# isl-org/lang-seg

Hardware: AMD Instinct MI355X
Metric: images/sec at 480x480, ViT-L/16 + 150 ADE20K labels (higher is better)
Workload: dtype fp16; 1 GPU; BASELINE configs[1]: clip_vitl16_384 LSegNet.forward, 480x480, K=150 ADE20K labels, text tower recomputed every call; per_gpu_batch=36, global_batch=36, labels=150, parallelism=dp1 (batch sharded, no collectives)

## Files before the change

lang-seg_amd/csrc/attention.hip:

```cpp
#include <cstdlib>
#include <type_traits>

#include "ops.h"
#include "../../include/lseg_hip.h"

namespace lseg {

struct AttnArgs {
    const uint16_t* q; const uint16_t* k; const uint16_t* vt;
    uint16_t* out;
    float* lse2;
    int B, H, ntok, npad, causal;
    float scale_log2e;
    int prescaled;
};

namespace {

#ifndef ATTN_PROBE
#define ATTN_PROBE(i)
#define ATTN_PROBE_DECL
#define ATTN_PROBE_DUMP
#endif

template <typename T, int NW, int NS, bool PRE>
__global__ __launch_bounds__(64 * NW, NW == 8 ? 2 : 3) void lseg_attention_kernel(const AttnArgs a) {
    extern __shared__ __attribute__((aligned(16))) char smem[];
    constexpr int TILE = 8192, STAGE = 2 * TILE;
    const int tid = threadIdx.x, lane = tid & 63;
    const int w = __builtin_amdgcn_readfirstlane(tid >> 6);
    const int hi = lane >> 5, ql = lane & 31;
    const int nqb = (a.ntok + 32 * NW - 1) / (32 * NW), BH = a.B * a.H;
    const int L = blockIdx.x;
    int qb = L % nqb, bh = L / nqb;
    if ((BH & 7) == 0) {
        const int xcd = L & 7, idx = L >> 3;
        qb = idx % nqb;
        bh = (idx / nqb) * 8 + xcd;
    }
    const int q0 = (qb * NW + w) * 32;
    const uint16_t* Q = a.q + (size_t)bh * a.npad * 64;
    const uint16_t* K = a.k + (size_t)bh * a.npad * 64;
    const uint16_t* Vt = a.vt + (size_t)bh * 64 * a.npad;

    i32x4_t qf[4];
    {
        int qr = q0 + ql;
        if (qr > a.npad - 1) qr = a.npad - 1;
#pragma unroll
        for (int ks = 0; ks < 4; ++ks)
            qf[ks] = *reinterpret_cast<const i32x4_t*>(Q + (size_t)qr * 64 + ks * 16 + hi * 8);
    }

    int kv_end = a.ntok;
    if (a.causal) {
        const int qend = (qb + 1) * 32 * NW;
        kv_end = qend < a.ntok ? qend : a.ntok;
    }
    const int n_tiles = (kv_end + 63) >> 6;

    constexpr int SPW = 8 / NW;
    uint32_t k_off[SPW], v_off[SPW];
#pragma unroll
    for (int s = 0; s < SPW; ++s) {
        const int r = (s * NW + w) * 8 + (lane >> 3);
        const int ch = ((lane & 7) ^ swz(r)) << 3;
        k_off[s] = (uint32_t)(r * 64 + ch) * 2u;
        v_off[s] = (uint32_t)(r * a.npad + ch) * 2u;
    }
    auto issue = [&](int t, int stage) {
        char* sk = smem + stage * STAGE;
        char* sv = sk + TILE;
        const char* kb = uniform_ptr(reinterpret_cast<const char*>(K + (size_t)t * 64 * 64));
        const char* vb = uniform_ptr(reinterpret_cast<const char*>(Vt + (size_t)t * 64));
#pragma unroll
        for (int s = 0; s < SPW; ++s) {
            uint32_t ko = k_off[s], vo = v_off[s];
            asm volatile("" : "+v"(ko), "+v"(vo));
            glds_slab_off(kb, ko, sk + (s * NW + w) * 1024);
            glds_slab_off(vb, vo, sv + (s * NW + w) * 1024);
        }
    };

    f32x16_t o[2];
#pragma unroll
    for (int d = 0; d < 2; ++d)
#pragma unroll
        for (int r = 0; r < 16; ++r) o[d][r] = 0.f;
    float m_run = PRE ? 0.f : -1e30f, l_run = 0.f;
    f32x16_t lacc;
#pragma unroll
    for (int r = 0; r < 16; ++r) lacc[r] = 0.f;
    const int one2 = std::is_same<T, F16>::value ? 0x3C003C00 : 0x3F803F80;
    const i32x4_t ones = {one2, one2, one2, one2};
    const int qrow = q0 + ql;
    const bool live = q0 < a.ntok;

    issue(0, 0);
    if (NS == 3 && n_tiles > 1) issue(1, 1);
    ATTN_PROBE_DECL
    int st_cur = 0, st_nxt = NS - 1;
    for (int t = 0; t < n_tiles; ++t) {
        if (NS == 3 && t + 1 < n_tiles) __builtin_amdgcn_s_waitcnt((2 * SPW) | (7 << 4));
        else __builtin_amdgcn_s_waitcnt(0);
        __syncthreads();
        ATTN_PROBE(0)
        if (t + NS - 1 < n_tiles) issue(t + NS - 1, st_nxt);
        const int st_use = st_cur;
        st_nxt = st_cur;
        st_cur = st_cur + 1 == NS ? 0 : st_cur + 1;
        if (!live) continue;
        ATTN_PROBE(1)
        const char* sk = smem + st_use * STAGE;
        const char* sv = sk + TILE;

        {
            i32x4_t kf[8];
#pragma unroll
            for (int ks = 0; ks < 4; ++ks)
#pragma unroll
                for (int sub = 0; sub < 2; ++sub)
                    kf[ks * 2 + sub] = *reinterpret_cast<const i32x4_t*>(sk + tile_off(sub * 32 + ql, ks * 2 + hi));
            __builtin_amdgcn_sched_barrier(0);
            f32x16_t s[2];
            const float s_init = PRE ? -m_run : 0.f;
#pragma unroll
            for (int sub = 0; sub < 2; ++sub)
#pragma unroll
                for (int r = 0; r < 16; ++r) s[sub][r] = s_init;
#pragma unroll
            for (int ks = 0; ks < 4; ++ks)
#pragma unroll
                for (int sub = 0; sub < 2; ++sub) s[sub] = mfma32<T>(kf[ks * 2 + sub], qf[ks], s[sub]);
            i32x4_t vf[8];
#pragma unroll
            for (int sub = 0; sub < 2; ++sub)
#pragma unroll
                for (int s2 = 0; s2 < 2; ++s2)
#pragma unroll
                    for (int d = 0; d < 2; ++d)
                        vf[(sub * 2 + s2) * 2 + d] = *reinterpret_cast<const i32x4_t*>(sv + tile_off(d * 32 + ql, sub * 4 + s2 * 2 + hi));
            __builtin_amdgcn_sched_barrier(0);
            ATTN_PROBE(2)
            const bool need_mask = a.causal || (t * 64 + 64 > a.ntok);
            if (need_mask) {
#pragma unroll
                for (int sub = 0; sub < 2; ++sub)
#pragma unroll
                    for (int r = 0; r < 16; ++r) {
                        const int key = t * 64 + sub * 32 + (r & 3) + 8 * (r >> 2) + 4 * hi;
                        const bool ok = key < a.ntok && (!a.causal || key <= qrow);
                        s[sub][r] = ok ? s[sub][r] : -INFINITY;
                    }
            }
            float mx = -INFINITY;
#pragma unroll
            for (int sub = 0; sub < 2; ++sub)
#pragma unroll
                for (int r = 0; r < 16; ++r) mx = fmaxf(mx, s[sub][r]);
            {
                const auto sw = __builtin_amdgcn_permlane32_swap(__float_as_uint(mx), __float_as_uint(mx), false, false);
                mx = fmaxf(__uint_as_float(sw[0]), __uint_as_float(sw[1]));
            }
            ATTN_PROBE(3)
            float lsum = 0.f;
            if constexpr (!PRE) {
                mx *= a.scale_log2e;
                const float m_new = fmaxf(m_run, mx);
                const bool grew = !__all(m_new == m_run);
                float alpha = 1.0f;
                if (grew) alpha = __builtin_amdgcn_exp2f(m_run - m_new);
                m_run = m_new;
#pragma unroll
                for (int sub = 0; sub < 2; ++sub)
#pragma unroll
                    for (int r = 0; r < 16; ++r) {
                        const float p = __builtin_amdgcn_exp2f(fmaf(s[sub][r], a.scale_log2e, -m_new));
                        s[sub][r] = p;
                        lsum += p;
                    }
                l_run = l_run * alpha + lsum;
                if (grew) {
#pragma unroll
                    for (int d = 0; d < 2; ++d)
#pragma unroll
                        for (int r = 0; r < 16; ++r) o[d][r] *= alpha;
                }
            } else {
                constexpr float THR = 8.0f;
                if (t == 0 || __any(mx > THR)) {
                    const float delta = t == 0 ? mx : fmaxf(mx, 0.f);
                    const float alpha = __builtin_amdgcn_exp2f(-delta);
                    m_run += delta;
#pragma unroll
                    for (int sub = 0; sub < 2; ++sub)
#pragma unroll
                        for (int r = 0; r < 16; ++r) s[sub][r] -= delta;
                    if (t > 0) {
#pragma unroll
                        for (int d = 0; d < 2; ++d)
#pragma unroll
                            for (int r = 0; r < 16; ++r) o[d][r] *= alpha;
#pragma unroll
                        for (int r = 0; r < 16; ++r) lacc[r] *= alpha;
                    }
                }
#pragma unroll
                for (int sub = 0; sub < 2; ++sub)
#pragma unroll
                    for (int r = 0; r < 16; ++r) {
                        s[sub][r] = __builtin_amdgcn_exp2f(s[sub][r]);
                    }
            }
            i32x4_t pf[2][2];
#pragma unroll
            for (int sub = 0; sub < 2; ++sub)
#pragma unroll
                for (int s2 = 0; s2 < 2; ++s2) {
                    const uint32_t a0 = pack2<T>(s[sub][8 * s2 + 0], s[sub][8 * s2 + 1]);
                    const uint32_t a1 = pack2<T>(s[sub][8 * s2 + 2], s[sub][8 * s2 + 3]);
                    const uint32_t b0 = pack2<T>(s[sub][8 * s2 + 4], s[sub][8 * s2 + 5]);
                    const uint32_t b1 = pack2<T>(s[sub][8 * s2 + 6], s[sub][8 * s2 + 7]);
                    const auto w0 = __builtin_amdgcn_permlane32_swap(a0, b0, false, false);
                    const auto w1 = __builtin_amdgcn_permlane32_swap(a1, b1, false, false);
                    pf[sub][s2][0] = (int)w0[0]; pf[sub][s2][1] = (int)w1[0];
                    pf[sub][s2][2] = (int)w0[1]; pf[sub][s2][3] = (int)w1[1];
                }
            ATTN_PROBE(4)
#pragma unroll
            for (int sub = 0; sub < 2; ++sub)
#pragma unroll
                for (int s2 = 0; s2 < 2; ++s2) {
#pragma unroll
                    for (int d = 0; d < 2; ++d) o[d] = mfma32<T>(vf[(sub * 2 + s2) * 2 + d], pf[sub][s2], o[d]);
                    if constexpr (PRE) lacc = mfma32<T>(ones, pf[sub][s2], lacc);
                }
        }
        ATTN_PROBE(5)
    }
    ATTN_PROBE_DUMP

    const float l_tot = PRE ? lacc[0] : l_run + __shfl_xor(l_run, 32);
    const float inv = 1.0f / l_tot;
    if (a.lse2 && hi == 0 && qrow < a.ntok) a.lse2[(size_t)bh * a.npad + qrow] = m_run + __builtin_amdgcn_logf(l_tot);
    if (qrow < a.ntok) {
        const int b = bh / a.H, h = bh - b * a.H;
        uint16_t* orow = a.out + ((size_t)b * a.ntok + qrow) * (a.H * 64) + h * 64;
#pragma unroll
        for (int d = 0; d < 2; ++d)
#pragma unroll
            for (int g = 0; g < 4; g += 2) {
                const uint32_t ax = pack2<T>(o[d][g * 4 + 0] * inv, o[d][g * 4 + 1] * inv), ay = pack2<T>(o[d][g * 4 + 2] * inv, o[d][g * 4 + 3] * inv);
                const uint32_t bx = pack2<T>(o[d][g * 4 + 4] * inv, o[d][g * 4 + 5] * inv), by = pack2<T>(o[d][g * 4 + 6] * inv, o[d][g * 4 + 7] * inv);
                const auto sx = __builtin_amdgcn_permlane32_swap(ax, bx, false, false);
                const auto sy = __builtin_amdgcn_permlane32_swap(ay, by, false, false);
                *reinterpret_cast<uint4*>(orow + d * 32 + (g + hi) * 8) = make_uint4(sx[0], sy[0], sx[1], sy[1]);
            }
    }
}

}

int launch_attention(const void* q, const void* k, const void* vt, void* out, int B, int H, int ntok,
                     int npad, int dtype, int causal, float scale, hipStream_t stream) {
    return launch_attention_lse(q, k, vt, out, nullptr, B, H, ntok, npad, dtype, causal, scale, stream);
}

int launch_attention_lse(const void* q, const void* k, const void* vt, void* out, float* lse2, int B, int H, int ntok,
                         int npad, int dtype, int causal, float scale, hipStream_t stream) {
    return launch_attention_ex(q, k, vt, out, lse2, B, H, ntok, npad, dtype, causal, scale, 0, stream);
}

int launch_attention_ex(const void* q, const void* k, const void* vt, void* out, float* lse2, int B, int H, int ntok,
                        int npad, int dtype, int causal, float scale, int prescaled, hipStream_t stream) {
    if (npad % 128 != 0 || npad < ntok) return set_error(LSEG_ERR_INVALID, "attention: npad=%d must be a multiple of 128 and >= ntok=%d", npad, ntok);
    if (prescaled && causal) return set_error(LSEG_ERR_UNSUPPORTED, "attention: the pre-scaled form has no causal variant");
    AttnArgs a;
    a.q = (const uint16_t*)q; a.k = (const uint16_t*)k; a.vt = (const uint16_t*)vt; a.out = (uint16_t*)out;
    a.lse2 = lse2;
    a.B = B; a.H = H; a.ntok = ntok; a.npad = npad; a.causal = causal;
    a.scale_log2e = scale * 1.4426950408889634f;
    a.prescaled = prescaled;
    if (dtype != DT_BF16 && dtype != DT_F16) return set_error(LSEG_ERR_INVALID, "attention: dtype %d", dtype);
    int dev = 0;
    LSEG_HIP_TRY(hipGetDevice(&dev));
    const bool narrow = (long)((ntok + 127) / 128) * B * H < 2L * device_cu_count(dev) && !causal;
    const int nw = narrow ? 2 : 4;
    const size_t lds = (size_t)2 * 2 * 8192;
    dim3 grid(((ntok + 32 * nw - 1) / (32 * nw)) * B * H);
#define ATT(TT, NWV, PV) hipLaunchKernelGGL((lseg_attention_kernel<TT, NWV, 2, PV>), grid, dim3(64 * NWV), lds, stream, a)
#define ATT_T(NWV, PV) do { if (dtype == DT_BF16) ATT(BF16, NWV, PV); else ATT(F16, NWV, PV); } while (0)
    if (nw == 2) { if (prescaled) ATT_T(2, true); else ATT_T(2, false); }
    else { if (prescaled) ATT_T(4, true); else ATT_T(4, false); }
#undef ATT_T
#undef ATT
    LSEG_HIP_TRY(hipGetLastError());
    return 0;
}

}
```

Baseline: 1085 images/sec.

## Add persistent 64-row-per-wave pre-scaled attention kernel with ping-pong softmax overlap

Adds a persistent attention kernel for the pre-scaled, non-causal path. Each wave owns 64 query rows as two 32-row halves, and the schedule interleaves one half's softmax/exp work with the other half's QK and PV MFMAs. K/V tiles are shared through a 3-stage LDS pipeline, and the running-max rescale is skipped unless the new max exceeds a threshold. It is selected when there are enough work items per CU, with an env override; the intent is to hide VALU softmax latency behind matrix work and halve K/V LDS reads per query row. In exchange it adds register pressure (launch bound of 1 block per CU), a larger LDS footprint and lazy-rescale numerics, and leaves compile-time ablation macros in the old kernel that are off by default.

```diff
diff --git a/lang-seg_amd/csrc/attention.hip b/lang-seg_amd/csrc/attention.hip
--- a/lang-seg_amd/csrc/attention.hip
+++ b/lang-seg_amd/csrc/attention.hip
@@ -16,6 +16,10 @@
 };
 
 namespace {
+
+#ifndef ATTN_ABL
+#define ATTN_ABL 0
+#endif
 
 #ifndef ATTN_PROBE
 #define ATTN_PROBE(i)
@@ -100,6 +104,9 @@
     if (NS == 3 && n_tiles > 1) issue(1, 1);
     ATTN_PROBE_DECL
     int st_cur = 0, st_nxt = NS - 1;
+#if ATTN_ABL == 3
+    i32x4_t kf_keep[8], vf_keep[8];
+#endif
     for (int t = 0; t < n_tiles; ++t) {
         if (NS == 3 && t + 1 < n_tiles) __builtin_amdgcn_s_waitcnt((2 * SPW) | (7 << 4));
         else __builtin_amdgcn_s_waitcnt(0);
@@ -116,11 +123,24 @@
 
         {
             i32x4_t kf[8];
+#if ATTN_ABL == 3
+            if (!PRE || t == 0)
+#endif
 #pragma unroll
             for (int ks = 0; ks < 4; ++ks)
 #pragma unroll
                 for (int sub = 0; sub < 2; ++sub)
                     kf[ks * 2 + sub] = *reinterpret_cast<const i32x4_t*>(sk + tile_off(sub * 32 + ql, ks * 2 + hi));
+#if ATTN_ABL == 3
+            if (PRE) {
+                if (t == 0) {
+#pragma unroll
+                    for (int i = 0; i < 8; ++i) kf_keep[i] = kf[i];
+                }
+#pragma unroll
+                for (int i = 0; i < 8; ++i) kf[i] = kf_keep[i];
+            }
+#endif
             __builtin_amdgcn_sched_barrier(0);
             f32x16_t s[2];
             const float s_init = PRE ? -m_run : 0.f;
@@ -133,6 +153,9 @@
 #pragma unroll
                 for (int sub = 0; sub < 2; ++sub) s[sub] = mfma32<T>(kf[ks * 2 + sub], qf[ks], s[sub]);
             i32x4_t vf[8];
+#if ATTN_ABL == 3
+            if (!PRE || t == 0)
+#endif
 #pragma unroll
             for (int sub = 0; sub < 2; ++sub)
 #pragma unroll
@@ -140,8 +163,22 @@
 #pragma unroll
                     for (int d = 0; d < 2; ++d)
                         vf[(sub * 2 + s2) * 2 + d] = *reinterpret_cast<const i32x4_t*>(sv + tile_off(d * 32 + ql, sub * 4 + s2 * 2 + hi));
+#if ATTN_ABL == 3
+            if (PRE) {
+                if (t == 0) {
+#pragma unroll
+                    for (int i = 0; i < 8; ++i) vf_keep[i] = vf[i];
+                }
+#pragma unroll
+                for (int i = 0; i < 8; ++i) vf[i] = vf_keep[i];
+            }
+#endif
             __builtin_amdgcn_sched_barrier(0);
             ATTN_PROBE(2)
+#if ATTN_ABL == 2 || ATTN_ABL == 3
+            if (PRE) asm volatile("" : "+v"(s[0]), "+v"(s[1]));
+            if (!PRE) {
+#endif
             const bool need_mask = a.causal || (t * 64 + 64 > a.ntok);
             if (need_mask) {
 #pragma unroll
@@ -209,10 +246,29 @@
                 for (int sub = 0; sub < 2; ++sub)
 #pragma unroll
                     for (int r = 0; r < 16; ++r) {
+#if ATTN_ABL == 1
+                        float e;
+                        asm("v_mov_b32 %0, %1" : "=v"(e) : "v"(s[sub][r]));
+                        s[sub][r] = e;
+#else
                         s[sub][r] = __builtin_amdgcn_exp2f(s[sub][r]);
+#endif
                     }
             }
+#if ATTN_ABL == 2 || ATTN_ABL == 3
+            }
+#endif
             i32x4_t pf[2][2];
+#if ATTN_ABL == 3
+            if (PRE) {
+#pragma unroll
+                for (int sub = 0; sub < 2; ++sub)
+#pragma unroll
+                    for (int s2 = 0; s2 < 2; ++s2)
+#pragma unroll
+                        for (int i = 0; i < 4; ++i) pf[sub][s2][i] = (int)__float_as_uint(s[sub][8 * s2 + i]);
+            } else
+#endif
 #pragma unroll
             for (int sub = 0; sub < 2; ++sub)
 #pragma unroll
@@ -233,7 +289,7 @@
                 for (int s2 = 0; s2 < 2; ++s2) {
 #pragma unroll
                     for (int d = 0; d < 2; ++d) o[d] = mfma32<T>(vf[(sub * 2 + s2) * 2 + d], pf[sub][s2], o[d]);
-                    if constexpr (PRE) lacc = mfma32<T>(ones, pf[sub][s2], lacc);
+                    if constexpr (PRE && ATTN_ABL != 4) lacc = mfma32<T>(ones, pf[sub][s2], lacc);
                 }
         }
         ATTN_PROBE(5)
@@ -259,7 +315,252 @@
     }
 }
 
-}
+__device__ __forceinline__ void attn_item_map(int item, int nqb, int BH, int& qb, int& bh) {
+    qb = item % nqb;
+    bh = item / nqb;
+    if ((BH & 7) == 0) {
+        const int xcd = item & 7, idx = item >> 3;
+        qb = idx % nqb;
+        bh = (idx / nqb) * 8 + xcd;
+    }
+}
+
+template <typename T>
+__device__ __forceinline__ void attn_qk(const i32x4_t (&kf)[8], const i32x4_t (&qf)[4], float m_run, f32x16_t (&s)[2]) {
+    const float s_init = -m_run;
+#pragma unroll
+    for (int sub = 0; sub < 2; ++sub)
+#pragma unroll
+        for (int r = 0; r < 16; ++r) s[sub][r] = s_init;
+#pragma unroll
+    for (int ks = 0; ks < 4; ++ks)
+#pragma unroll
+        for (int sub = 0; sub < 2; ++sub) s[sub] = mfma32<T>(kf[ks * 2 + sub], qf[ks], s[sub]);
+}
+
+template <typename T>
+__device__ __forceinline__ void attn_pv(const i32x4_t (&vf)[8], const i32x4_t (&pf)[2][2], const i32x4_t ones, f32x16_t (&o)[2],
+                                        f32x16_t& lacc) {
+#pragma unroll
+    for (int sub = 0; sub < 2; ++sub)
+#pragma unroll
+        for (int s2 = 0; s2 < 2; ++s2) {
+#pragma unroll
+            for (int d = 0; d < 2; ++d) o[d] = mfma32<T>(vf[(sub * 2 + s2) * 2 + d], pf[sub][s2], o[d]);
+            lacc = mfma32<T>(ones, pf[sub][s2], lacc);
+        }
+}
+
+template <bool MASK>
+__device__ __forceinline__ void attn_pre_decide(f32x16_t (&s)[2], float& m_run, f32x16_t (&o)[2], f32x16_t& lacc, int t, int ntok, int hi) {
+    if (MASK) {
+#pragma unroll
+        for (int sub = 0; sub < 2; ++sub)
+#pragma unroll
+            for (int r = 0; r < 16; ++r) {
+                const int key = t * 64 + sub * 32 + (r & 3) + 8 * (r >> 2) + 4 * hi;
+                s[sub][r] = key < ntok ? s[sub][r] : -INFINITY;
+            }
+    }
+    float mx = -INFINITY;
+#pragma unroll
+    for (int sub = 0; sub < 2; ++sub)
+#pragma unroll
+        for (int r = 0; r < 16; ++r) mx = fmaxf(mx, s[sub][r]);
+    {
+        const auto sw = __builtin_amdgcn_permlane32_swap(__float_as_uint(mx), __float_as_uint(mx), false, false);
+        mx = fmaxf(__uint_as_float(sw[0]), __uint_as_float(sw[1]));
+    }
+    constexpr float THR = 8.0f;
+    if (t == 0 || __any(mx > THR)) {
+        const float delta = t == 0 ? mx : fmaxf(mx, 0.f);
+        const float alpha = __builtin_amdgcn_exp2f(-delta);
+        m_run += delta;
+#pragma unroll
+        for (int sub = 0; sub < 2; ++sub)
+#pragma unroll
+            for (int r = 0; r < 16; ++r) s[sub][r] -= delta;
+        if (t > 0) {
+#pragma unroll
+            for (int d = 0; d < 2; ++d)
+#pragma unroll
+                for (int r = 0; r < 16; ++r) o[d][r] *= alpha;
+#pragma unroll
+            for (int r = 0; r < 16; ++r) lacc[r] *= alpha;
+        }
+    }
+}
+template <typename T>
+__device__ __forceinline__ void attn_pre_finish(f32x16_t (&s)[2], i32x4_t (&pf)[2][2]) {
+#pragma unroll
+    for (int sub = 0; sub < 2; ++sub)
+#pragma unroll
+        for (int r = 0; r < 16; ++r) s[sub][r] = __builtin_amdgcn_exp2f(s[sub][r]);
+#pragma unroll
+    for (int sub = 0; sub < 2; ++sub)
+#pragma unroll
+        for (int s2 = 0; s2 < 2; ++s2) {
+            const uint32_t a0 = pack2<T>(s[sub][8 * s2 + 0], s[sub][8 * s2 + 1]);
+            const uint32_t a1 = pack2<T>(s[sub][8 * s2 + 2], s[sub][8 * s2 + 3]);
+            const uint32_t b0 = pack2<T>(s[sub][8 * s2 + 4], s[sub][8 * s2 + 5]);
+            const uint32_t b1 = pack2<T>(s[sub][8 * s2 + 6], s[sub][8 * s2 + 7]);
+            const auto w0 = __builtin_amdgcn_permlane32_swap(a0, b0, false, false);
+            const auto w1 = __builtin_amdgcn_permlane32_swap(a1, b1, false, false);
+            pf[sub][s2][0] = (int)w0[0]; pf[sub][s2][1] = (int)w1[0];
+            pf[sub][s2][2] = (int)w0[1]; pf[sub][s2][3] = (int)w1[1];
+        }
+}
+
+template <typename T>
+__device__ __forceinline__ void attn_pre_store(const AttnArgs& a, const f32x16_t (&o)[2], const f32x16_t& lacc, float m_run, int bh, int qrow,
+                                               int hi) {
+    const float l_tot = lacc[0];
+    const float inv = 1.0f / l_tot;
+    if (a.lse2 && hi == 0 && qrow < a.ntok) a.lse2[(size_t)bh * a.npad + qrow] = m_run + __builtin_amdgcn_logf(l_tot);
+    if (qrow < a.ntok) {
+        const int b = bh / a.H, h = bh - b * a.H;
+        uint16_t* orow = a.out + ((size_t)b * a.ntok + qrow) * (a.H * 64) + h * 64;
+#pragma unroll
+        for (int d = 0; d < 2; ++d)
+#pragma unroll
+            for (int g = 0; g < 4; g += 2) {
+                const uint32_t ax = pack2<T>(o[d][g * 4 + 0] * inv, o[d][g * 4 + 1] * inv), ay = pack2<T>(o[d][g * 4 + 2] * inv, o[d][g * 4 + 3] * inv);
+                const uint32_t bx = pack2<T>(o[d][g * 4 + 4] * inv, o[d][g * 4 + 5] * inv), by = pack2<T>(o[d][g * 4 + 6] * inv, o[d][g * 4 + 7] * inv);
+                const auto sx = __builtin_amdgcn_permlane32_swap(ax, bx, false, false);
+                const auto sy = __builtin_amdgcn_permlane32_swap(ay, by, false, false);
+                *reinterpret_cast<uint4*>(orow + d * 32 + (g + hi) * 8) = make_uint4(sx[0], sy[0], sx[1], sy[1]);
+            }
+    }
+}
+
+template <typename T>
+__global__ __launch_bounds__(256, 1) void lseg_attention_pre_w64_kernel(const AttnArgs a, const int n_items) {
+    extern __shared__ __attribute__((aligned(16))) char smem[];
+    constexpr int TILE = 8192, STAGE = 2 * TILE, NS = 3;
+    const int tid = threadIdx.x, lane = tid & 63;
+    const int w = __builtin_amdgcn_readfirstlane(tid >> 6);
+    const int hi = lane >> 5, ql = lane & 31;
+    const int nqb = (a.ntok + 255) >> 8, BH = a.B * a.H;
+    const int n_tiles = (a.ntok + 63) >> 6;
+
+    uint32_t k_off[2], v_off[2];
+#pragma unroll
+    for (int s = 0; s < 2; ++s) {
+        const int r = (s * 4 + w) * 8 + (lane >> 3);
+        const int ch = ((lane & 7) ^ swz(r)) << 3;
+        k_off[s] = (uint32_t)(r * 64 + ch) * 2u;
+        v_off[s] = (uint32_t)(r * a.npad + ch) * 2u;
+    }
+    const int one2 = std::is_same<T, F16>::value ? 0x3C003C00 : 0x3F803F80;
+    const i32x4_t ones = {one2, one2, one2, one2};
+
+    for (int item = blockIdx.x; item < n_items; item += gridDim.x) {
+        int qb, bh;
+        attn_item_map(item, nqb, BH, qb, bh);
+        const int q0 = qb * 256 + w * 64;
+        const uint16_t* Q = a.q + (size_t)bh * a.npad * 64;
+        const uint16_t* K = a.k + (size_t)bh * a.npad * 64;
+        const uint16_t* Vt = a.vt + (size_t)bh * 64 * a.npad;
+        auto issue = [&](int t) {
+            char* sk = smem + (t % NS) * STAGE;
+            char* sv = sk + TILE;
+            const char* kb = uniform_ptr(reinterpret_cast<const char*>(K + (size_t)t * 64 * 64));
+            const char* vb = uniform_ptr(reinterpret_cast<const char*>(Vt + (size_t)t * 64));
+#pragma unroll
+            for (int s = 0; s < 2; ++s) {
+                uint32_t ko = k_off[s], vo = v_off[s];
+                asm volatile("" : "+v"(ko), "+v"(vo));
+                glds_slab_off(kb, ko, sk + (s * 4 + w) * 1024);
+                glds_slab_off(vb, vo, sv + (s * 4 + w) * 1024);
+            }
+        };
+        auto barrier_tile = [&](int j) {
+            if (j + 1 < n_tiles) __builtin_amdgcn_s_waitcnt(4 | (7 << 4));
+            else __builtin_amdgcn_s_waitcnt(0);
+            __syncthreads();
+            if (j + 2 < n_tiles) issue(j + 2);
+        };
+
+        i32x4_t qfA[4], qfB[4];
+        {
+            int ra = q0 + ql, rb = q0 + 32 + ql;
+            if (ra > a.npad - 1) ra = a.npad - 1;
+            if (rb > a.npad - 1) rb = a.npad - 1;
+#pragma unroll
+            for (int ks = 0; ks < 4; ++ks) {
+                qfA[ks] = *reinterpret_cast<const i32x4_t*>(Q + (size_t)ra * 64 + ks * 16 + hi * 8);
+                qfB[ks] = *reinterpret_cast<const i32x4_t*>(Q + (size_t)rb * 64 + ks * 16 + hi * 8);
+            }
+        }
+        issue(0);
+        if (n_tiles > 1) issue(1);
+        barrier_tile(0);
+
+        if (q0 >= a.ntok) {
+            for (int j = 1; j < n_tiles; ++j) barrier_tile(j);
+        } else {
+            f32x16_t oA[2], oB[2], lA, lB, sA[2], sB[2];
+#pragma unroll
+            for (int r = 0; r < 16; ++r) {
+                oA[0][r] = 0.f; oA[1][r] = 0.f; oB[0][r] = 0.f; oB[1][r] = 0.f; lA[r] = 0.f; lB[r] = 0.f;
+            }
+            float mA = 0.f, mB = 0.f;
+            i32x4_t kf[8], vf[8], pA[2][2], pB[2][2];
+            auto read_k = [&](int t) {
+                const char* sk = smem + (t % NS) * STAGE;
+#pragma unroll
+                for (int ks = 0; ks < 4; ++ks)
+#pragma unroll
+                    for (int sub = 0; sub < 2; ++sub)
+                        kf[ks * 2 + sub] = *reinterpret_cast<const i32x4_t*>(sk + tile_off(sub * 32 + ql, ks * 2 + hi));
+            };
+            auto read_v = [&](int t) {
+                const char* sv = smem + (t % NS) * STAGE + TILE;
+#pragma unroll
+                for (int sub = 0; sub < 2; ++sub)
+#pragma unroll
+                    for (int s2 = 0; s2 < 2; ++s2)
+#pragma unroll
+                        for (int d = 0; d < 2; ++d)
+                            vf[(sub * 2 + s2) * 2 + d] = *reinterpret_cast<const i32x4_t*>(sv + tile_off(d * 32 + ql, sub * 4 + s2 * 2 + hi));
+            };
+            auto tile = [&](int t, auto first, auto last) {
+                constexpr bool LAST = decltype(last)::value;
+                attn_pre_decide<LAST>(sA, mA, oA, lA, t, a.ntok, hi);
+                if constexpr (!decltype(first)::value) attn_pv<T>(vf, pB, ones, oB, lB);
+                read_v(t);
+                attn_qk<T>(kf, qfB, mB, sB);
+                attn_pre_finish<T>(sA, pA);
+                if constexpr (!LAST) {
+                    barrier_tile(t + 1);
+                    read_k(t + 1);
+                }
+                attn_pre_decide<LAST>(sB, mB, oB, lB, t, a.ntok, hi);
+                attn_pv<T>(vf, pA, ones, oA, lA);
+                if constexpr (!LAST) attn_qk<T>(kf, qfA, mA, sA);
+                attn_pre_finish<T>(sB, pB);
+            };
+            using yes = std::true_type;
+            using no = std::false_type;
+            read_k(0);
+            attn_qk<T>(kf, qfA, mA, sA);
+            if (n_tiles == 1) tile(0, yes{}, yes{});
+            else {
+                tile(0, yes{}, no{});
+                for (int t = 1; t + 1 < n_tiles; ++t) tile(t, no{}, no{});
+                tile(n_tiles - 1, no{}, yes{});
+            }
+            attn_pv<T>(vf, pB, ones, oB, lB);
+            attn_pre_store<T>(a, oA, lA, mA, bh, q0 + ql, hi);
+            attn_pre_store<T>(a, oB, lB, mB, bh, q0 + 32 + ql, hi);
+        }
+        __syncthreads();
+    }
+}
+
+}
+
+constexpr int PRE_W64_MIN_ITEMS_PER_CU = 2;
 
 int launch_attention(const void* q, const void* k, const void* vt, void* out, int B, int H, int ntok,
                      int npad, int dtype, int causal, float scale, hipStream_t stream) {
@@ -269,6 +570,12 @@
 int launch_attention_lse(const void* q, const void* k, const void* vt, void* out, float* lse2, int B, int H, int ntok,
                          int npad, int dtype, int causal, float scale, hipStream_t stream) {
     return launch_attention_ex(q, k, vt, out, lse2, B, H, ntok, npad, dtype, causal, scale, 0, stream);
+}
+
+static bool use_pre_w64(long n_items, int cus) {
+    static const int impl = getenv("LSEG_ATTN_IMPL") ? atoi(getenv("LSEG_ATTN_IMPL")) : -1;
+    if (impl >= 0) return impl == 1;
+    return n_items >= (long)PRE_W64_MIN_ITEMS_PER_CU * cus;
 }
 
 int launch_attention_ex(const void* q, const void* k, const void* vt, void* out, float* lse2, int B, int H, int ntok,
@@ -284,6 +591,16 @@
     if (dtype != DT_BF16 && dtype != DT_F16) return set_error(LSEG_ERR_INVALID, "attention: dtype %d", dtype);
     int dev = 0;
     LSEG_HIP_TRY(hipGetDevice(&dev));
+    const int cus = device_cu_count(dev);
+    if (prescaled && use_pre_w64(B * H * ((ntok + 255) / 256), cus)) {
+        const int n_items = B * H * ((ntok + 255) / 256);
+        const int g = n_items < cus ? n_items : cus - cus % 8;
+        const size_t lds3 = (size_t)3 * 2 * 8192;
+        if (dtype == DT_BF16) hipLaunchKernelGGL(lseg_attention_pre_w64_kernel<BF16>, dim3(g), dim3(256), lds3, stream, a, n_items);
+        else hipLaunchKernelGGL(lseg_attention_pre_w64_kernel<F16>, dim3(g), dim3(256), lds3, stream, a, n_items);
+        LSEG_HIP_TRY(hipGetLastError());
+        return 0;
+    }
     const bool narrow = (long)((ntok + 127) / 128) * B * H < 2L * device_cu_count(dev) && !causal;
     const int nw = narrow ? 2 : 4;
     const size_t lds = (size_t)2 * 2 * 8192;
```

After: 1010 images/sec (median of 2 runs). -6.9%, worse.
